# BBischof/ESRecsys

Measured on AMD Instinct MI355X. Metric: training pairs/sec, higher is better.
Workload: dtype f32; 1 GPU; inbatch: V=1000000 x D=128 fp32 tables, B=8192, sparse Adagrad; score_precision=auto -> f16x2, ids=uniform, parallelism=single

## Files before the change

esrecsys_amd/csrc/esr_inbatch2h.hip:

```cpp
#include "esr_inbatch_mfma.h"
#include <atomic>
#include <type_traits>
#include <time.h>

namespace esr {

typedef _Float16 f16x8 __attribute__((ext_vector_type(8)));
typedef _Float16 f16x2 __attribute__((ext_vector_type(2)));

constexpr int kHLseOff = 2 * kPlaneBytes;
constexpr int kHBufBytes = kHLseOff + 4 * 256;
constexpr float kHOptHead = 4.0f;
constexpr float kHOverflow = 60000.0f;
constexpr int kHBufs = 3;
constexpr float kHPexp = 14.0f;
constexpr float kHBoundSafe = 14.0f;
constexpr int kHScaleWords = 8;

#define H_MFMA(a, b, c) __builtin_amdgcn_mfma_f32_32x32x16_f16((a), (b), (c), 0, 0, 0)
#define H_SB() __builtin_amdgcn_sched_barrier(0)
#define H_DMA_BARRIER()                                 \
  {                                                     \
    asm volatile("s_waitcnt vmcnt(0)" ::: "memory");    \
    __syncthreads();                                    \
// ... 219 lines not shown
    const float4 f = rowsrc_load4(X, grow, d0 + 4 * q);
    v[4 * q] = f.x; v[4 * q + 1] = f.y; v[4 * q + 2] = f.z; v[4 * q + 3] = f.w;
  }
  {
    float ss = 0.f;
#pragma unroll
    for (int e = 0; e < 16; ++e) ss = fmaf(v[e], v[e], ss);
    ss += __shfl_xor(ss, 1, 64);
    ss += __shfl_xor(ss, 2, 64);
    ss += __shfl_xor(ss, 4, 64);
    ss = fmaxf(ss, __shfl_xor(ss, 8, 64));
    ss = fmaxf(ss, __shfl_xor(ss, 16, 64));
    ss = fmaxf(ss, __shfl_xor(ss, 32, 64));
    if ((t & 63) == 0) nrm[((int64_t)blockIdx.y * gridDim.x + chunk) * 4 + (t >> 6)] = ss;
  }
  f16x8 p[2][2];
#pragma unroll
  for (int e = 0; e < 16; ++e) {
    const float xs = v[e] * mul;
    const _Float16 a = (_Float16)xs;
    const _Float16 b = (_Float16)(xs - (float)a);
    p[0][e >> 3][e & 7] = a;
    p[1][e >> 3][e & 7] = b;
  }
#pragma unroll
  for (int pl = 0; pl < 2; ++pl) {
    f16x8* dst = reinterpret_cast<f16x8*>(R + ((int64_t)pl * B + grow) * k3D + d0);
    dst[0] = p[pl][0];
    dst[1] = p[pl][1];
  }
}

constexpr unsigned long long kPollTicks = 300000000ull;
__device__ __forceinline__ unsigned amax_code(float amax) {
  if (!(amax > 0.f)) return 0u;
  if (!(amax < INFINITY)) return 255u;
  int x;
  frexpf(amax, &x);
  return (unsigned)min(max(x + 127, 1), 254);
}
__device__ __forceinline__ int scale_exp_code(unsigned code) {
  if (code == 0u || code == 255u) return 0;
  const int e = 14 - ((int)code - 127);
  return e < -100 ? -100 : (e > 100 ? 100 : e);
}

__global__ __launch_bounds__(256) void prepsplit2h_kernel(RowSrc X0, RowSrc X1, int64_t B, _Float16* __restrict__ R0,
                                                         _Float16* __restrict__ R1,
                                                         unsigned long long* __restrict__ ent,
                                                         unsigned long long token, float* __restrict__ diag,
                                                         float* __restrict__ nrm, float* __restrict__ sc,
                                                         unsigned long long* __restrict__ loss_acc,
                                                         int* __restrict__ flags, int nflags,
                                                         float* __restrict__ copy0, float* __restrict__ copy1,
                                                         unsigned* __restrict__ czero, int two_level) {
  __shared__ float red[8];
  __shared__ unsigned cred[8];
  const int t = threadIdx.x, chunk = blockIdx.x, nchunks = gridDim.x;
  if (chunk == 0 && t <= kLossWords) {
    loss_acc[t * 16] = 0ull;
    if (t == 0) loss_acc[8] = 0ull;
  }
  if (chunk == 1 || nchunks == 1)
    for (int i = t; i < nflags; i += 256) flags[i] = 0;
  if (czero && chunk == 0 && t < 16) czero[t] = 0u;
  const int row = t >> 3, d0 = (t & 7) * 16;
  const int64_t grow = (int64_t)chunk * 32 + row;
  float vq[16], vc[16];
  {
    const int64_t rq = X0.idx ? (int64_t)X0.idx[grow] : grow;
    const int64_t rc = X1.idx ? (int64_t)X1.idx[grow] : grow;
    RowSrc Y0 = X0, Y1 = X1;
    Y0.idx = nullptr; Y1.idx = nullptr;
#pragma unroll
    for (int q = 0; q < 4; ++q) {
      const float4 f = rowsrc_load4(Y0, rq, d0 + 4 * q);
      const float4 g = rowsrc_load4(Y1, rc, d0 + 4 * q);
      vq[4 * q] = f.x; vq[4 * q + 1] = f.y; vq[4 * q + 2] = f.z; vq[4 * q + 3] = f.w;
      vc[4 * q] = g.x; vc[4 * q + 1] = g.y; vc[4 * q + 2] = g.z; vc[4 * q + 3] = g.w;
      if (copy0 && d0 + 4 * q < X0.ld) *reinterpret_cast<float4*>(copy0 + grow * X0.ld + d0 + 4 * q) = f;
      if (copy1 && d0 + 4 * q < X1.ld) *reinterpret_cast<float4*>(copy1 + grow * X1.ld + d0 + 4 * q) = g;
    }
  }
  float mq = 0.f, mc = 0.f, dot = 0.f, ssq = 0.f, ssc = 0.f;
#pragma unroll
  for (int e = 0; e < 16; ++e) {
    mq = fmaxf(mq, fabsf(vq[e]));
    mc = fmaxf(mc, fabsf(vc[e]));
    dot = fmaf(vq[e], vc[e], dot);
    ssq = fmaf(vq[e], vq[e], ssq);
    ssc = fmaf(vc[e], vc[e], ssc);
  }
  dot += __shfl_xor(dot, 1, 64); dot += __shfl_xor(dot, 2, 64); dot += __shfl_xor(dot, 4, 64);
  ssq += __shfl_xor(ssq, 1, 64); ssq += __shfl_xor(ssq, 2, 64); ssq += __shfl_xor(ssq, 4, 64);
  ssc += __shfl_xor(ssc, 1, 64); ssc += __shfl_xor(ssc, 2, 64); ssc += __shfl_xor(ssc, 4, 64);
  if ((t & 7) == 0) diag[grow] = dot;
#pragma unroll
  for (int o = 8; o < 64; o <<= 1) {
    ssq = fmaxf(ssq, __shfl_xor(ssq, o, 64));
    ssc = fmaxf(ssc, __shfl_xor(ssc, o, 64));
  }
  if ((t & 63) == 0) {
    nrm[((int64_t)0 * nchunks + chunk) * 4 + (t >> 6)] = ssq;
    nrm[((int64_t)1 * nchunks + chunk) * 4 + (t >> 6)] = ssc;
  }
#pragma unroll
  for (int o = 32; o > 0; o >>= 1) {
    mq = fmaxf(mq, __shfl_xor(mq, o, 64));
    mc = fmaxf(mc, __shfl_xor(mc, o, 64));
  }
  if ((t & 63) == 0) { red[t >> 6] = mq; red[4 + (t >> 6)] = mc; }
  __syncthreads();
  if (t == 0) {
    mq = fmaxf(fmaxf(red[0], red[1]), fmaxf(red[2], red[3]));
    mc = fmaxf(fmaxf(red[4], red[5]), fmaxf(red[6], red[7]));
    __hip_atomic_store(&ent[chunk], (token << 16) | (unsigned long long)(amax_code(mq) << 8 | amax_code(mc)),
                       __ATOMIC_RELAXED, __HIP_MEMORY_SCOPE_AGENT);
  }
  unsigned cq = 0u, cc = 0u;
  bool timed_out = false;
  const unsigned long long t_start = __builtin_amdgcn_s_memrealtime();
  const bool gatherer = chunk == 0 || !two_level;
  for (int i = gatherer ? t : (t == 0 ? nchunks : nchunks + 1); i < (gatherer ? nchunks : nchunks + 1); i += 256) {
    unsigned long long v;
    while (((v = __hip_atomic_load(&ent[i], __ATOMIC_RELAXED, __HIP_MEMORY_SCOPE_AGENT)) >> 16) != token) {
      if (__builtin_amdgcn_s_memrealtime() - t_start > kPollTicks) { timed_out = true; break; }
      __builtin_amdgcn_s_sleep(4);
    }
    cq = max(cq, (unsigned)(v >> 8) & 255u);
    cc = max(cc, (unsigned)v & 255u);
  }
  if (timed_out) atomicOr(reinterpret_cast<unsigned*>(loss_acc + 8), 1u);
#pragma unroll
  for (int o = 32; o > 0; o >>= 1) {
    cq = max(cq, (unsigned)__shfl_xor((int)cq, o, 64));
    cc = max(cc, (unsigned)__shfl_xor((int)cc, o, 64));
  }
  if ((t & 63) == 0) { cred[t >> 6] = cq; cred[4 + (t >> 6)] = cc; }
  __syncthreads();
  cq = max(max(cred[0], cred[1]), max(cred[2], cred[3]));
  cc = max(max(cred[4], cred[5]), max(cred[6], cred[7]));
  if (two_level && chunk == 0 && t == 0)
    __hip_atomic_store(&ent[nchunks], (token << 16) | (unsigned long long)(cq << 8 | cc), __ATOMIC_RELAXED,
                       __HIP_MEMORY_SCOPE_AGENT);
  const int eq = scale_exp_code(cq), ec = scale_exp_code(cc);
  if (chunk == 0 && t == 0) {
    sc[0] = ldexpf(1.f, -(eq + ec));
    sc[1] = ldexpf(1.f, -ec);
    sc[2] = ldexpf(1.f, -(eq + (int)kHPexp));
    sc[3] = ldexpf(1.f, eq);
// ... 228 lines not shown
    _Pragma("unroll") for (int g_ = 0; g_ < 2; ++g_) {                                                    \
      const u32x4 u_ = {pw[q_][4 * g_], pw[q_][4 * g_ + 1], pw[q_][4 * g_ + 2], pw[q_][4 * g_ + 3]};      \
      pb[q_][g_] = __builtin_bit_cast(f16x8, u_);                                                         \
    }
#define H_O_PHASE(DMA_ON, DBUF)                                                                           \
  {                                                                                                       \
    H_PB();                                                                                               \
    H_TR_WAIT();     \
    H_SB(); H_O_ROW(1, 0, 0); H_SB(); H_O_G1(0, 3); if (DMA_ON) { H_DP(0, g0, DBUF); }                    \
    H_SB(); H_O_ROW(0, 1, 0); H_SB(); H_O_G1(3, 6); if (DMA_ON) { H_DP(1, g1, DBUF); }                    \
    H_SB(); H_O_ROW(0, 0, 0); H_SB(); H_O_G1(6, 8); if (DMA_ON) { H_DP(2, g2, DBUF); }                    \
    H_TR_WAIT();                                                                                          \
    H_SB(); H_O_ROW(1, 0, 1); H_SB(); if (DMA_ON) { H_DP(3, g3, DBUF); }                                  \
    H_SB(); H_O_ROW(0, 1, 1); H_SB();                                                                     \
    H_SB(); H_O_ROW(0, 0, 1); H_SB();                                                                     \
    if (DMA_ON) H_DMA_ADVANCE();                                                                          \
  }
#define H_TR_BASES(BUF)                                                                                   \
  {                                                                                                       \
    const uint32_t slot_ = (uint32_t)((BUF) - lds);                                                       \
    _Pragma("unroll") for (int db_ = 0; db_ < 4; ++db_) { trc_[db_][0] = trb_[db_][0] + slot_; trc_[db_][1] = trb_[db_][1] + slot_; } \
  }
#define H_TR_SETUP()                                                                                      \
  const int tr_a = (lane & 15) >> 2;                                                                      \
  const int tr_e = (2 * ((lane >> 4) & 1)) + ((lane & 3) >> 1), tr_low = (lane & 1) * 8;                  \
  const int tr_row0 = (4 * h + tr_a) * 256, tr_row1 = (4 * h + 8 + tr_a) * 256;                           \
  const int tr_l0 = ((tr_e ^ (h & 3)) << 4) | tr_low, tr_l1 = ((tr_e ^ ((h + 2) & 3)) << 4) | tr_low;     \
  uint32_t trb_[4][2], trc_[4][2];                                                                        \
  _Pragma("unroll") for (int db = 0; db < 4; ++db) {                                                      \
    trb_[db][0] = (uint32_t)(uintptr_t)(__attribute__((address_space(3))) const char*)lds + tr_row0 + (((db ^ tr_a) << 6) | tr_l0); \
    trb_[db][1] = (uint32_t)(uintptr_t)(__attribute__((address_space(3))) const char*)lds + tr_row1 + (((db ^ tr_a) << 6) | tr_l1); \
  }

template <int KIND>
__global__ ESR_NO_PK __launch_bounds__(256) __attribute__((amdgpu_waves_per_eu(2, 2))) void inbatch2h_q_kernel(const _Float16* __restrict__ Xr, const _Float16* __restrict__ Yr,
                                                         int64_t B, int nsplit, float sl2_in,
                                                         const float* __restrict__ sc, const float* __restrict__ ref,
                                                         int nsplit_ref, const float* __restrict__ diag, int mode,
                                                         int* __restrict__ flags, float* __restrict__ part_m,
                                                         float* __restrict__ part_O, float* __restrict__ part_l,
                                                         float* __restrict__ Pmat) {
  __shared__ __attribute__((aligned(16))) char lds[kHBufs * kHBufBytes];
  if (KIND == 1 && flags[blockIdx.x] == 0) return;
  H_TIMING_DECL();
  int t = threadIdx.x, lane = t & 63;
  const int w = __builtin_amdgcn_readfirstlane(t >> 6);
  int j = lane & 31, h = lane >> 5;
  H_TR_SETUP();
  const uint32_t lds32 = (uint32_t)(uintptr_t)(__attribute__((address_space(3))) const char*)lds;
  (void)lds32;
  const int ob = blockIdx.x / nsplit, split = blockIdx.x % nsplit;
  const int64_t xrow = (int64_t)ob * k3Owned + w * 32 + j;
  const int nc = (int)(B / k3Chunk) / nsplit;
  const int64_t c0 = (int64_t)split * nc;
  const int64_t nch = B / 32;
  const float sl2 = sl2_in * sc[0];

  char* pst_u = nullptr;
  const uint32_t pst_v = (uint32_t)((((j >> 3) * 16) + ((2 * h + ((j >> 2) & 1)) * 4) + (j & 3)) * 16);
#if defined(H_PROBE_Q_NOSTORE)
#define H_P_ST(M, V0, V1, V2, V3)
#else
#define H_P_ST(M, V0, V1, V2, V3) \
  __builtin_nontemporal_store(u32x4{(V0), (V1), (V2), (V3)}, reinterpret_cast<u32x4*>(pst_u + (M) * 1024 + pst_v))
#endif

  f32x16 acc[4];
  f32x2 l2 = {0.f, 0.f};
  int dpos = 0;
  const char* const baseY = reinterpret_cast<const char*>(Yr);
  uint32_t g0 = 0, g1 = 0, g2 = 0, g3 = 0;
  f16x8 bx[2][8];
#pragma unroll
  for (int p = 0; p < 2; ++p)
// ... 123 lines not shown
      const f16x2 pq = pk_f16(resid_lo(e0, pa), resid_hi(e1, pa));
      pw[0][s] = __builtin_bit_cast(uint32_t, pa);
      pw[1][s] = __builtin_bit_cast(uint32_t, pq);
    }
#pragma unroll
    for (int m2 = 0; m2 < 2; ++m2)
#pragma unroll
      for (int pl = 0; pl < 2; ++pl) {
        H_P_ST(2 * m2 + pl, pw[pl][4 * m2], pw[pl][4 * m2 + 1], pw[pl][4 * m2 + 2], pw[pl][4 * m2 + 3]);
      }
    H_O_PHASE(false, lds);
  }
  };
  if (KIND == 1) {
    sweep(std::true_type{});
  } else {
    sweep(std::false_type{});
    if (KIND == 2 && mode != 0 && __syncthreads_or((mode == 2 || !(emax <= kHOverflow)) ? 1 : 0)) {
      asm volatile("" : "+v"(t), "+v"(lane), "+v"(j), "+v"(h));
      sweep(std::true_type{});
    }
  }
#undef H_P_ST
  H_TIMING_WRITE(H_TIMING_Q);
  float* orow = part_O + ((int64_t)split * B + xrow) * k3D;
#pragma unroll
  for (int db = 0; db < 4; ++db)
#pragma unroll
    for (int q = 0; q < 4; ++q)
      *reinterpret_cast<float4*>(orow + 32 * db + 8 * q + 4 * h) =
          make_float4(acc[db][4 * q], acc[db][4 * q + 1], acc[db][4 * q + 2], acc[db][4 * q + 3]);
  const float l = l2[0] + l2[1];
  const float ltot = l + __shfl_xor(l, 32, 64);
  if (h == 0) part_l[(int64_t)split * B + xrow] = ltot;
  if (KIND == 0 && (mode == 2 || !(emax <= kHOverflow))) flags[blockIdx.x] = 1;
}

template <int K>
__device__ __forceinline__ uint32_t dmah8_off0(int64_t B, int64_t chunk, int t) {
  const int row = t >> 4, seg = (t & 15) ^ swz16(row);
  return (uint32_t)((((int64_t)K * B + chunk * 32 + row) * k3D + seg * 8) * 2);
}
constexpr int kH1Waves = 8, kH1Owned = 32 * kH1Waves;
constexpr int kH1BufBytes = kPlaneBytes + kH1Waves * 256;
#define H1_DP(K, G, BUF) dmah_piece<K>(baseY, G, (BUF), w)
#define H1_DMA_REF(BUF)                                                                                   \
  __builtin_amdgcn_global_load_lds((gptr_t)(ref + (c0 + dpos) * 32 + (lane & 31)),                        \
                                   (lptr_t)((BUF) + kPlaneBytes + w * 256), 4, 0, 0)
#define H1_DMA_ADVANCE()                                                                   \
  {                                                                                        \
    const uint32_t step_ = (dpos + 1 == nc) ? (uint32_t)(8192 - nc * 8192) : 8192u;        \
    dpos = (dpos + 1 == nc) ? 0 : dpos + 1;                                                \
    g0 += step_;                                                                           \
  }
#define H1_DMA_CHUNK(BUF) { if (!QSIDE) { H1_DMA_REF(BUF); } H1_DP(0, g0, BUF); H1_DMA_ADVANCE(); }
#define H1_LOAD_REFS(BUF)                                                                                 \
  if (!QSIDE) {                                                                                           \
    f16x8 raw_[4];                                                                                        \
    _Pragma("unroll") for (int m_ = 0; m_ < 4; ++m_)                                                      \
      raw_[m_] = lds_b128<0>(lds32 + (uint32_t)((BUF) - lds) + (uint32_t)(kPlaneBytes + w * 256 + (8 * m_ + 4 * h) * 4)); \
    H_TR_WAIT();                                                                                          \
    _Pragma("unroll") for (int m_ = 0; m_ < 4; ++m_) {                                                    \
      const float4 lv_ = __builtin_bit_cast(float4, raw_[m_]);                                            \
      rf[4 * m_] = kHPexp - lv_.x; rf[4 * m_ + 1] = kHPexp - lv_.y;                                       \
      rf[4 * m_ + 2] = kHPexp - lv_.z; rf[4 * m_ + 3] = kHPexp - lv_.w;                                   \
    }                                                                                                     \
  }
// ... 641 lines not shown
                                                   float* __restrict__ lse_nat = nullptr) {
  const int64_t row = (int64_t)blockIdx.x * 256 + threadIdx.x;
  if (row >= B) return;
  float pm[8], pl[8];
#pragma unroll
  for (int s = 0; s < 8; ++s) {
    pm[s] = -INFINITY; pl[s] = 0.f;
    if (s < nsplit) {
      pm[s] = part_m[(int64_t)s * B + row];
      pl[s] = part_l[(int64_t)s * B + row];
    }
  }
  float M = pm[0], L = 0.f;
  float wt[8];
#pragma unroll
  for (int s = 1; s < 8; ++s) M = fmaxf(M, pm[s]);
#pragma unroll
  for (int s = 0; s < 8; ++s) {
    wt[s] = pm[s] == M ? 1.f : __builtin_amdgcn_exp2f(pm[s] - M);
    L = __fmaf_rn(pl[s], wt[s], L);
  }
  const float invL1 = __fdiv_rn(1.0f, L);
#pragma unroll
  for (int s = 0; s < 8; ++s)
    if (s < nsplit) fac[(int64_t)s * B + row] = __fmul_rn(__fmul_rn(invL1, invl_scale), wt[s]);
  if (lse2) {
    const float l2v = __fadd_rn(M, __builtin_amdgcn_logf(L));
    lse2[row] = l2v;
    if (lse_nat) lse_nat[row] = l2v * k3Ln2;
  }
}

constexpr int kCtExpShift = 11;
__global__ __launch_bounds__(256) void facscale2h_kernel(RowSrc X, int64_t B, int nsplit,
                                                        const float* __restrict__ part_m,
                                                        const float* __restrict__ part_l, float invl_scale,
                                                        const float* __restrict__ sc, float* __restrict__ fac,
                                                        float* __restrict__ lse2, float* __restrict__ lse_nat,
                                                        _Float16* __restrict__ Yt, int* __restrict__ cflags) {
  const int t = threadIdx.x, chunk = blockIdx.x;
  const int row = t >> 3, sl = t & 7, d0 = sl * 16;
  const int64_t grow = (int64_t)chunk * 32 + row;
  float v[16];
  {
    const int64_t r = X.idx ? (int64_t)X.idx[grow] : grow;
    RowSrc Y0 = X;
    Y0.idx = nullptr;
#pragma unroll
    for (int q = 0; q < 4; ++q) {
      const float4 f = rowsrc_load4(Y0, r, d0 + 4 * q);
      v[4 * q] = f.x; v[4 * q + 1] = f.y; v[4 * q + 2] = f.z; v[4 * q + 3] = f.w;
    }
  }
  const float pm_l = sl < nsplit ? part_m[(int64_t)sl * B + grow] : -INFINITY;
  const float pl_l = sl < nsplit ? part_l[(int64_t)sl * B + grow] : 0.f;
  float pm[8], pl[8];
  const int lane0 = (t & 63) & ~7;
#pragma unroll
  for (int s = 0; s < 8; ++s) {
    pm[s] = __shfl(pm_l, lane0 + s, 64);
    pl[s] = __shfl(pl_l, lane0 + s, 64);
  }
  float M = pm[0], L = 0.f;
  float wt[8];
#pragma unroll
  for (int s = 1; s < 8; ++s) M = fmaxf(M, pm[s]);
#pragma unroll
  for (int s = 0; s < 8; ++s) {
    wt[s] = pm[s] == M ? 1.f : __builtin_amdgcn_exp2f(pm[s] - M);
    L = __fmaf_rn(pl[s], wt[s], L);
  }
  const float invL1 = __fdiv_rn(1.0f, L);
  const float f1 = __fmul_rn(invL1, invl_scale);
  float wmine = 1.f;
#pragma unroll
  for (int s = 0; s < 8; ++s) wmine = s == sl ? wt[s] : wmine;
  const float fs = __fmul_rn(f1, wmine);
  if (sl < nsplit) {
    fac[(int64_t)sl * B + grow] = fs;
    if (fs != f1) cflags[sl] = 1;
  }
  if (sl == 0 && lse2) {
    const float l2v = __fadd_rn(M, __builtin_amdgcn_logf(L));
    lse2[grow] = l2v;
    if (lse_nat) lse_nat[grow] = l2v * k3Ln2;
  }
  const float mul = sc[3] * ldexpf(1.f, -kCtExpShift);
  float m = 0.f;
  f16x8 p[2][2];
#pragma unroll
  for (int e = 0; e < 16; ++e) {
    const float xs = __fmul_rn(v[e], f1) * mul;
    m = fmaxf(m, fabsf(xs));
    const _Float16 a = (_Float16)xs;
    const _Float16 b = (_Float16)(xs - (float)a);
    p[0][e >> 3][e & 7] = a;
    p[1][e >> 3][e & 7] = b;
  }
  m = fmaxf(m, __shfl_xor(m, 1, 64));
  m = fmaxf(m, __shfl_xor(m, 2, 64));
  m = fmaxf(m, __shfl_xor(m, 4, 64));
  if (sl < nsplit && (!(m < 60000.f) || (f1 != 0.f && m < kCtLive))) cflags[sl] = 1;
#pragma unroll
  for (int pl2 = 0; pl2 < 2; ++pl2) {
    f16x8* dst = reinterpret_cast<f16x8*>(Yt + ((int64_t)pl2 * B + grow) * k3D + d0);
    dst[0] = p[pl2][0];
    dst[1] = p[pl2][1];
  }
}

struct InbatchHWs {
  _Float16 *Qh, *Ch;
  float *part_O, *part_O2, *fac_side, *Qcopy, *Ccopy, *part_m, *part_mr, *part_l, *lse2, *fac, *Pmat, *nrm, *amax, *sc, *diag;
  int* flags;
  unsigned long long* loss_acc;
  unsigned long long* ent;
  _Float16* Qt;
  unsigned* czero;
  int* cflags;
};
constexpr int64_t kHMaxB = 16384;

static size_t inbatch2h_ws_layout(int64_t B, char* base, InbatchHWs* ws) {
  size_t off = 0;
  auto take = [&](size_t bytes) {
    char* p = base ? base + off : nullptr;
    off += align_up(bytes, 256);
    return p;
  };
  const size_t planes = (size_t)2 * B * k3D * 2;
  InbatchHWs w;
  w.Qh = (_Float16*)take(planes);
  w.Ch = (_Float16*)take(planes);
  w.part_O = (float*)take((size_t)8 * B * k3D * 4);
  w.part_O2 = (float*)take((size_t)8 * B * k3D * 4);
  w.fac_side = (float*)take((size_t)8 * B * 4);
  w.Qcopy = (float*)take((size_t)B * k3D * 4);
  w.Ccopy = (float*)take((size_t)B * k3D * 4);
  w.part_m = (float*)take((size_t)8 * B * 4);
  w.part_mr = (float*)take((size_t)8 * B * 4);
  w.part_l = (float*)take((size_t)8 * B * 4);
  w.lse2 = (float*)take((size_t)B * 4);
  w.fac = (float*)take((size_t)8 * B * 4);
  w.diag = (float*)take((size_t)B * 4);
  w.flags = (int*)take((size_t)8 * (B / k3Owned) * sizeof(int));
  w.Pmat = (float*)take((size_t)B * B * 4);
  w.loss_acc = (unsigned long long*)take(sizeof(unsigned long long) * 16 * (1 + kLossWords));
  w.nrm = (float*)take((size_t)2 * (B / k3Chunk) * 4 * sizeof(float));
  w.amax = (float*)take((size_t)2 * (B / k3Chunk) * sizeof(float));
  w.sc = (float*)take(kHScaleWords * sizeof(float));
  w.ent = (unsigned long long*)take((size_t)(B / k3Chunk + 1) * sizeof(unsigned long long));
  w.Qt = (_Float16*)take(planes);
  w.czero = (unsigned*)take(16 * sizeof(unsigned));
  w.cflags = reinterpret_cast<int*>(w.czero ? w.czero + 8 : nullptr);
  if (ws) *ws = w;
  return off;
}

static int inbatch2h_nsplit(int64_t B, int per_cu) {
  const int64_t owned_blocks = B / k3Owned, nchunks = B / k3Chunk;
  int best = 1;
  for (int s = 1; s <= 8; ++s)
    if (nchunks % s == 0 && owned_blocks * s <= 320 * per_cu) best = s;
  return best;
}

struct InbatchUpdate {
  void* tables[2];
  float* accums[2];
  int64_t row_offsets[3];
  int dtype;
  const int32_t* sorted_vids;
  const int32_t* perm;
  float* grad_rows;
  float lr, eps;
  bool skip_long;
};

int inbatch_merge_update(void* const* tables, float* const* accums, const int64_t* row_offsets, int dtype,
                         const int32_t* sorted_vids, const int32_t* perm, const InbatchMergeArgs& a, float lr, float eps,
                         hipStream_t st);
int sparse_adagrad_range(void* const* tables, float* const* accums, const int64_t* row_offsets, int ntables, int dtype,
                         int D, const int32_t* sorted_vids, const int32_t* perm, int64_t n, float* grad_rows, float lr,
                         float eps, bool skip_long, hipStream_t st);

static bool inbatch_events(hipEvent_t* fork, hipEvent_t* join) {
  constexpr int kMaxDev = 16;
// ... 65 lines not shown
  const int pc_blocks = (int)cdiv(B, kCtOwned);
  int nsplit_c = 1;
  for (int sp = 1; sp <= 8; ++sp)
    if (nchunks % sp == 0 && pc_blocks * sp <= 320) nsplit_c = sp;
  const int grid_c = pc_blocks * nsplit_c;
  const int grid_q = (int)(B / k3Owned) * nsplit_q;
  const int mgrid = (int)std::min<int64_t>(k3MergeBlocks, cdiv(B, kBlock / 32));
  const char* refe = getenv("ESR_IB2H_REF");
  const int mode = (refe && refe[0] == 'r' && refe[1] == 'o') ? 0 : ((refe && refe[0] == 'r' && refe[1] == 'e') ? 2 : 1);
  const char* fe = getenv("ESR_IB2H_FUSED");
  const bool fused = !(fe && fe[0] == '0') && mode != 0;
  int nsplit_r = 1;
  hipEvent_t ev_fork = nullptr, ev_join = nullptr;
  const char* b16e = getenv("ESR_IB2H_BF16");
  const bool one_plane = fused && ((Qs.bf16 && Cs.bf16 && !(b16e && b16e[0] == 't')) || (b16e && b16e[0] == 'f'));
  const bool overlapped = fused && !one_plane && side != nullptr && side != st && inbatch_events(&ev_fork, &ev_join);
  const char* mue = getenv("ESR_IB2H_MERGE_UPDATE");
  const bool merge_upd = fused && !overlapped && upd != nullptr && upd->skip_long && D == k3D && Qs.ld == k3D &&
                         Cs.ld == k3D && !(mue && mue[0] == '0');
  auto merging_update = [&](int nsplit_of_c, const float* part_O_of_c) -> int {
    InbatchMergeArgs a;
    a.part_O[0] = ws.part_O; a.part_O[1] = part_O_of_c;
    a.nsplit[0] = nsplit_q; a.nsplit[1] = nsplit_of_c;
    a.oscale[0] = ws.sc + 1; a.oscale[1] = ws.sc + 2;
    a.partner[0] = ws.Ccopy; a.partner[1] = ws.Qcopy;
    a.part_m = ws.part_m; a.part_l = ws.part_l;
    a.B = B;
    a.scale = scale; a.lam = regularization; a.inv_bs = inv_bs;
    a.loss_acc = ws.loss_acc; a.loss_scale = 1.0 / (double)batch_size; a.loss_out = loss;
    a.zero_words = ws.ent; a.nzero = nchunks + 1;
    return inbatch_merge_update(upd->tables, upd->accums, upd->row_offsets, upd->dtype, upd->sorted_vids, upd->perm, a,
                                upd->lr, upd->eps, st);
  };
  if (fused) {
    static std::atomic<unsigned long long> call_seq{0};
    static const unsigned long long seed =
        (unsigned long long)(uintptr_t)&call_seq ^ (unsigned long long)time(nullptr) * 0x9E3779B97F4A7C15ull;
    unsigned long long z = seed + 0x9E3779B97F4A7C15ull * (call_seq.fetch_add(1) + 1);
    z = (z ^ (z >> 30)) * 0xBF58476D1CE4E5B9ull;
    z = (z ^ (z >> 27)) * 0x94D049BB133111EBull;
    const unsigned long long token = ((z ^ (z >> 31)) >> 16) | 1ull;
    const char* tle = getenv("ESR_IB2H_POLL");
    const int two_level = (tle && tle[0] == 'f') ? 0 : 1;
    ESR_KT("prepsplit2h_kernel", st,
           hipLaunchKernelGGL(prepsplit2h_kernel, dim3(nchunks), dim3(256), 0, st, Qs, Cs, B, ws.Qh, ws.Ch, ws.ent, token,
                              ws.diag, ws.nrm, ws.sc, ws.loss_acc, ws.flags, grid_q, (overlapped || merge_upd) ? ws.Qcopy : (float*)nullptr,
                              (overlapped || merge_upd) ? ws.Ccopy : (float*)nullptr, ws.czero, two_level));
    if (one_plane) {
      const int blocks1 = (int)cdiv(B, kH1Owned);
      int nsplit_1 = 1;
      for (int sp = 1; sp <= 8; ++sp)
        if (nchunks % sp == 0 && blocks1 * sp <= 320) nsplit_1 = sp;
      const int nsplit_q = nsplit_1, grid_q = blocks1 * nsplit_1;
      const char* dbg1h = getenv("ESR_IB1H_DBG");
      if (dbg1h && dbg1h[0] == '1') {
        hipLaunchKernelGGL((inbatch1h_kernel<true, 1>), dim3(grid_q), dim3(512), 0, st, (const _Float16*)ws.Qh,
                           (const _Float16*)ws.Ch, B, nsplit_q, sl2, (const float*)ws.sc, (const float*)ws.diag,
                           (const float*)nullptr, mode, ws.part_m, ws.part_O, ws.part_l);
      } else
      ESR_KT("inbatch1h_kernel_q", st,
             hipLaunchKernelGGL((inbatch1h_kernel<true>), dim3(grid_q), dim3(512), 0, st, (const _Float16*)ws.Qh,
                                (const _Float16*)ws.Ch, B, nsplit_q, sl2, (const float*)ws.sc, (const float*)ws.diag,
                                (const float*)nullptr, mode, ws.part_m, ws.part_O, ws.part_l));
      if (merge_upd) {
        ESR_KT("fac2h_kernel", st,
               hipLaunchKernelGGL(fac2h_kernel, dim3((unsigned)cdiv(B, 256)), dim3(256), 0, st, B, nsplit_q,
                                  (const float*)ws.part_m, (const float*)ws.part_l, ldexpf(1.f, (int)kHPexp), ws.fac,
                                  ws.lse2, lse));
      } else
      ESR_KT("inbatch3_merge_kernel_q", st,
             hipLaunchKernelGGL((inbatch3_merge_kernel<true>), dim3(mgrid), dim3(kBlock), 0, st, Qs, Cs, gq_rows, B,
                                nsplit_q, (const float*)ws.part_O, (const float*)ws.part_m, (const float*)ws.part_l, scale,
                                regularization, inv_bs, ws.lse2, lse, gQ, ws.loss_acc, 1.0 / (double)batch_size, loss,
                                (float*)nullptr, (const float*)(ws.sc + 1), ldexpf(1.f, (int)kHPexp), ws.fac));
      float* const part_O_1c = merge_upd ? ws.part_O2 : ws.part_O;
      if (dbg1h && (dbg1h[0] == '1' || dbg1h[0] == '2')) {
        hipLaunchKernelGGL((inbatch1h_kernel<false, 1>), dim3(grid_q), dim3(512), 0, st, (const _Float16*)ws.Ch,
                           (const _Float16*)ws.Qh, B, nsplit_q, sl2, (const float*)ws.sc, (const float*)nullptr,
                           (const float*)ws.lse2, mode, (float*)nullptr, part_O_1c, (float*)nullptr);
      } else
      ESR_KT("inbatch1h_kernel_c", st,
             hipLaunchKernelGGL((inbatch1h_kernel<false>), dim3(grid_q), dim3(512), 0, st, (const _Float16*)ws.Ch,
                                (const _Float16*)ws.Qh, B, nsplit_q, sl2, (const float*)ws.sc, (const float*)nullptr,
                                (const float*)ws.lse2, mode, (float*)nullptr, part_O_1c, (float*)nullptr));
      if (merge_upd) return merging_update(nsplit_q, part_O_1c);
      ESR_KT("inbatch3_merge_kernel_c", st,
             hipLaunchKernelGGL((inbatch3_merge_kernel<false>), dim3(mgrid), dim3(kBlock), 0, st, Cs, Qs, gc_rows, B,
                                nsplit_q, (const float*)ws.part_O, (const float*)ws.part_m, (const float*)ws.part_l, scale,
                                regularization, inv_bs, ws.lse2, (float*)nullptr, gC, ws.loss_acc,
                                1.0 / (double)batch_size, loss, (float*)nullptr, (const float*)(ws.sc + 2), 1.0f,
                                (float*)nullptr, ws.ent, nchunks + 1));
      if (upd) {
        const int rc = sparse_adagrad_range(upd->tables, upd->accums, upd->row_offsets, 2, upd->dtype, D, upd->sorted_vids,
                                            upd->perm, 2 * B, upd->grad_rows, upd->lr, upd->eps, upd->skip_long, st);
        if (rc != ESR_OK) return rc;
      }
      return check_launch(who);
    }
    ESR_KT("inbatch2h_q_kernel", st,
           hipLaunchKernelGGL((inbatch2h_q_kernel<2>), dim3(grid_q), dim3(256), 0, st, (const _Float16*)ws.Qh,
                              (const _Float16*)ws.Ch, B, nsplit_q, sl2, (const float*)ws.sc, (const float*)ws.part_mr, 1,
                              (const float*)ws.diag, mode, ws.flags, ws.part_m, ws.part_O, ws.part_l, ws.Pmat));
  } else {
  ESR_KT("prep2h_kernel", st, hipLaunchKernelGGL(prep2h_kernel, dim3(nchunks), dim3(256), 0, st, Qs, Cs, ws.amax, ws.diag));
  ESR_KT("split2h_kernel", st,
         hipLaunchKernelGGL(split2h_kernel, dim3(nchunks, 2), dim3(256), 0, st, Qs, Cs, B, ws.Qh, ws.Ch,
                            (const float*)ws.amax, ws.nrm, ws.sc, ws.loss_acc, ws.flags, grid_q));
  if (mode == 0) {
    const int rm_blocks = (int)cdiv(B, kHRmOwned);
    for (int sp = 1; sp <= 8; ++sp)
      if (nchunks % sp == 0 && rm_blocks * sp <= 320) nsplit_r = sp;
    ESR_KT("rowmax2h_kernel", st,
           hipLaunchKernelGGL(rowmax2h_kernel, dim3(rm_blocks * nsplit_r), dim3(256), 0, st, (const _Float16*)ws.Qh,
                              (const _Float16*)ws.Ch, B, nsplit_r, sl2, (const float*)ws.nrm, (const float*)ws.sc,
                              ws.part_mr));
  }
  {
    ESR_KT("inbatch2h_q_kernel", st,
           hipLaunchKernelGGL((inbatch2h_q_kernel<0>), dim3(grid_q), dim3(256), 0, st, (const _Float16*)ws.Qh,
                              (const _Float16*)ws.Ch, B, nsplit_q, sl2, (const float*)ws.sc, (const float*)ws.part_mr,
                              nsplit_r, (const float*)ws.diag, mode, ws.flags, ws.part_m, ws.part_O, ws.part_l, ws.Pmat));
    if (mode != 0)
      ESR_KT("inbatch2h_q_kernel_redo", st,
             hipLaunchKernelGGL((inbatch2h_q_kernel<1>), dim3(grid_q), dim3(256), 0, st, (const _Float16*)ws.Qh,
                                (const _Float16*)ws.Ch, B, nsplit_q, sl2, (const float*)ws.sc, (const float*)ws.part_mr,
                                nsplit_r, (const float*)ws.diag, mode, ws.flags, ws.part_m, ws.part_O, ws.part_l, ws.Pmat));
  }
  }
  hipStream_t st_q = overlapped ? side : st;
  float* const part_O_c = (overlapped || merge_upd) ? ws.part_O2 : ws.part_O;
  const RowSrc Qm = overlapped ? RowSrc{ws.Qcopy, nullptr, 0, Qs.ld} : Qs;
  const RowSrc Cm = overlapped ? RowSrc{ws.Ccopy, nullptr, 0, Cs.ld} : Cs;
  const int nc_q = nchunks / nsplit_q;
  const char* pcm = getenv("ESR_IB2H_PC");
  const int force_general = (!fused || (pcm && pcm[0] == 'g')) ? 1 : 0;
  if (overlapped) {
    if (hipEventRecord(ev_fork, st) != hipSuccess || hipStreamWaitEvent(side, ev_fork, 0) != hipSuccess) {
      set_error("%s: could not fork the side stream", who);
      return ESR_ELAUNCH;
    }
  }
  if (!force_general)
    ESR_KT("facscale2h_kernel", st,
           hipLaunchKernelGGL(facscale2h_kernel, dim3(nchunks), dim3(256), 0, st,
                              (overlapped || merge_upd) ? RowSrc{ws.Qcopy, nullptr, 0, Qs.ld} : Qs, B, nsplit_q,
                              (const float*)ws.part_m, (const float*)ws.part_l, ldexpf(1.f, (int)kHPexp),
                              (const float*)ws.sc, ws.fac, merge_upd ? ws.lse2 : (float*)nullptr,
                              merge_upd ? lse : (float*)nullptr, ws.Qt, ws.cflags));
  else if (overlapped || merge_upd)
    ESR_KT("fac2h_kernel", st,
           hipLaunchKernelGGL(fac2h_kernel, dim3((unsigned)cdiv(B, 256)), dim3(256), 0, st, B, nsplit_q,
                              (const float*)ws.part_m, (const float*)ws.part_l, ldexpf(1.f, (int)kHPexp), ws.fac,
                              merge_upd ? ws.lse2 : (float*)nullptr, merge_upd ? lse : (float*)nullptr));
  if (!merge_upd)
  ESR_KT("inbatch3_merge_kernel_q", st_q,
         hipLaunchKernelGGL((inbatch3_merge_kernel<true>), dim3(mgrid), dim3(kBlock), 0, st_q, Qm, Cm, gq_rows, B, nsplit_q,
                            (const float*)ws.part_O, (const float*)ws.part_m, (const float*)ws.part_l, scale,
                            regularization, inv_bs, ws.lse2, lse, gQ, ws.loss_acc, 1.0 / (double)batch_size, loss,
                            (float*)nullptr, (const float*)(ws.sc + 1), ldexpf(1.f, (int)kHPexp),
                            overlapped ? ws.fac_side : ws.fac));
  if (overlapped) {
    if (upd) {
      const int rc = sparse_adagrad_range(upd->tables, upd->accums, upd->row_offsets, 2, upd->dtype, D, upd->sorted_vids,
                                          upd->perm, B, upd->grad_rows, upd->lr, upd->eps, upd->skip_long, side);
      if (rc != ESR_OK) return rc;
    }
    if (hipEventRecord(ev_join, side) != hipSuccess) {
      set_error("%s: could not record the join event", who);
      return ESR_ELAUNCH;
    }
  }
  ESR_KT("inbatch2h_pct_kernel", st,
         hipLaunchKernelGGL(inbatch2h_pct_kernel, dim3(grid_c), dim3(512), 0, st, (const _Float16*)ws.Qt,
                            (const _Float16*)ws.Qh, B, nsplit_c, (const float*)ws.fac, nc_q, (const char*)ws.Pmat,
                            ldexpf(1.f, kCtExpShift), (const int*)ws.cflags, force_general, part_O_c));
// ... 138 lines not shown
```

Baseline: 38.60 million pairs/s.

## Fuse facscale into q-kernel epilogue via arrival counter; defer prep copies

Adds an optional epilogue to the in-batch q kernel. Each split block publishes its partial max and sum, then bumps a per-row-group arrival counter, and the last block to arrive computes the softmax factors and the scaled f16 Q planes itself. This removes the separate facscale kernel launch. Independently, the prep kernel now writes its fp32 row copies after publishing the amax entry instead of during the loads, which shortens the path to the cross-block poll but keeps the values live in registers longer. The fused epilogue is opt-in through an environment variable and adds zeroed counter words to the workspace.

Result: no change. 38.63 million pairs/s, median of 2 (+0.1%).

```diff
diff --git a/esrecsys_amd/csrc/esr_inbatch2h.hip b/esrecsys_amd/csrc/esr_inbatch2h.hip
--- a/esrecsys_amd/csrc/esr_inbatch2h.hip
+++ b/esrecsys_amd/csrc/esr_inbatch2h.hip
@@ -275,6 +275,9 @@
 }
 
 constexpr unsigned long long kPollTicks = 300000000ull;
+constexpr int64_t kHMaxB = 16384;
+constexpr int kHZeroWords = 16 + (int)(kHMaxB / k3Owned);
+static_assert(kHZeroWords <= 256, "one thread per zeroed word");
 __device__ __forceinline__ unsigned amax_code(float amax) {
   if (!(amax > 0.f)) return 0u;
   if (!(amax < INFINITY)) return 255u;
@@ -296,7 +299,7 @@
                                                          unsigned long long* __restrict__ loss_acc,
                                                          int* __restrict__ flags, int nflags,
                                                          float* __restrict__ copy0, float* __restrict__ copy1,
-                                                         unsigned* __restrict__ czero, int two_level) {
+                                                         unsigned* __restrict__ czero, int two_level, int copy_late) {
   __shared__ float red[8];
   __shared__ unsigned cred[8];
   const int t = threadIdx.x, chunk = blockIdx.x, nchunks = gridDim.x;
@@ -306,7 +309,7 @@
   }
   if (chunk == 1 || nchunks == 1)
     for (int i = t; i < nflags; i += 256) flags[i] = 0;
-  if (czero && chunk == 0 && t < 16) czero[t] = 0u;
+  if (czero && chunk == 0 && t < kHZeroWords) czero[t] = 0u;
   const int row = t >> 3, d0 = (t & 7) * 16;
   const int64_t grow = (int64_t)chunk * 32 + row;
   float vq[16], vc[16];
@@ -321,8 +324,10 @@
       const float4 g = rowsrc_load4(Y1, rc, d0 + 4 * q);
       vq[4 * q] = f.x; vq[4 * q + 1] = f.y; vq[4 * q + 2] = f.z; vq[4 * q + 3] = f.w;
       vc[4 * q] = g.x; vc[4 * q + 1] = g.y; vc[4 * q + 2] = g.z; vc[4 * q + 3] = g.w;
-      if (copy0 && d0 + 4 * q < X0.ld) *reinterpret_cast<float4*>(copy0 + grow * X0.ld + d0 + 4 * q) = f;
-      if (copy1 && d0 + 4 * q < X1.ld) *reinterpret_cast<float4*>(copy1 + grow * X1.ld + d0 + 4 * q) = g;
+      if (!copy_late) {
+        if (copy0 && d0 + 4 * q < X0.ld) *reinterpret_cast<float4*>(copy0 + grow * X0.ld + d0 + 4 * q) = f;
+        if (copy1 && d0 + 4 * q < X1.ld) *reinterpret_cast<float4*>(copy1 + grow * X1.ld + d0 + 4 * q) = g;
+      }
     }
   }
   float mq = 0.f, mc = 0.f, dot = 0.f, ssq = 0.f, ssc = 0.f;
@@ -359,6 +364,17 @@
     mc = fmaxf(fmaxf(red[4], red[5]), fmaxf(red[6], red[7]));
     __hip_atomic_store(&ent[chunk], (token << 16) | (unsigned long long)(amax_code(mq) << 8 | amax_code(mc)),
                        __ATOMIC_RELAXED, __HIP_MEMORY_SCOPE_AGENT);
+  }
+  if (copy_late) {
+#pragma unroll
+    for (int q = 0; q < 4; ++q) {
+      if (copy0 && d0 + 4 * q < X0.ld)
+        *reinterpret_cast<float4*>(copy0 + grow * X0.ld + d0 + 4 * q) =
+            make_float4(vq[4 * q], vq[4 * q + 1], vq[4 * q + 2], vq[4 * q + 3]);
+      if (copy1 && d0 + 4 * q < X1.ld)
+        *reinterpret_cast<float4*>(copy1 + grow * X1.ld + d0 + 4 * q) =
+            make_float4(vc[4 * q], vc[4 * q + 1], vc[4 * q + 2], vc[4 * q + 3]);
+    }
   }
   unsigned cq = 0u, cc = 0u;
   bool timed_out = false;
@@ -653,14 +669,24 @@
     trb_[db][1] = (uint32_t)(uintptr_t)(__attribute__((address_space(3))) const char*)lds + tr_row1 + (((db ^ tr_a) << 6) | tr_l1); \
   }
 
-template <int KIND>
+struct FacEpi {
+  unsigned* arrive;
+  const float* X;
+  float invl_scale;
+  float *fac, *lse2, *lse_nat;
+  _Float16* Yt;
+  int* cflags;
+};
+static __device__ void facscale2h_block(FacEpi e, int t, int ob, int64_t B, int nsplit, const float* part_m,
+                                        const float* part_l, const float* __restrict__ sc);
+template <int KIND, bool EPI = false>
 __global__ ESR_NO_PK __launch_bounds__(256) __attribute__((amdgpu_waves_per_eu(2, 2))) void inbatch2h_q_kernel(const _Float16* __restrict__ Xr, const _Float16* __restrict__ Yr,
                                                          int64_t B, int nsplit, float sl2_in,
                                                          const float* __restrict__ sc, const float* __restrict__ ref,
                                                          int nsplit_ref, const float* __restrict__ diag, int mode,
                                                          int* __restrict__ flags, float* __restrict__ part_m,
                                                          float* __restrict__ part_O, float* __restrict__ part_l,
-                                                         float* __restrict__ Pmat) {
+                                                         float* __restrict__ Pmat, FacEpi epi) {
   __shared__ __attribute__((aligned(16))) char lds[kHBufs * kHBufBytes];
   if (KIND == 1 && flags[blockIdx.x] == 0) return;
   H_TIMING_DECL();
@@ -850,7 +876,22 @@
           make_float4(acc[db][4 * q], acc[db][4 * q + 1], acc[db][4 * q + 2], acc[db][4 * q + 3]);
   const float l = l2[0] + l2[1];
   const float ltot = l + __shfl_xor(l, 32, 64);
-  if (h == 0) part_l[(int64_t)split * B + xrow] = ltot;
+  const bool arrive = KIND == 2 && EPI;
+  const int te = w * 64 + h * 32 + j;
+  unsigned arrived = 0u;
+  if (arrive) {
+    if (h == 0) {
+      __hip_atomic_store(&part_m[(int64_t)split * B + xrow], -nrefv[0], __ATOMIC_RELAXED, __HIP_MEMORY_SCOPE_AGENT);
+      __hip_atomic_store(&part_l[(int64_t)split * B + xrow], ltot, __ATOMIC_RELAXED, __HIP_MEMORY_SCOPE_AGENT);
+    }
+    asm volatile("s_waitcnt vmcnt(0)" ::: "memory");
+    __syncthreads();
+    if (te == 0) arrived = __hip_atomic_fetch_add(&epi.arrive[ob], 1u, __ATOMIC_RELAXED, __HIP_MEMORY_SCOPE_AGENT) + 1u;
+  } else if (h == 0) {
+    part_l[(int64_t)split * B + xrow] = ltot;
+  }
+  if (arrive && __syncthreads_or(arrived == (unsigned)nsplit ? 1 : 0))
+    facscale2h_block(epi, te, ob, B, nsplit, part_m, part_l, sc);
   if (KIND == 0 && (mode == 2 || !(emax <= kHOverflow))) flags[blockIdx.x] = 1;
 }
 
@@ -1558,6 +1599,67 @@
 }
 
 constexpr int kCtExpShift = 11;
+__device__ __forceinline__ void facscale2h_row(const float (&v)[16], float pm_l, float pl_l, int t, int sl, int64_t grow,
+                                               int64_t B, int nsplit, float invl_scale, const float* __restrict__ sc,
+                                               float* __restrict__ fac, float* __restrict__ lse2,
+                                               float* __restrict__ lse_nat, _Float16* __restrict__ Yt,
+                                               int* __restrict__ cflags) {
+  const int d0 = sl * 16;
+  float pm[8], pl[8];
+  const int lane0 = (t & 63) & ~7;
+#pragma unroll
+  for (int s = 0; s < 8; ++s) {
+    pm[s] = __shfl(pm_l, lane0 + s, 64);
+    pl[s] = __shfl(pl_l, lane0 + s, 64);
+  }
+  float M = pm[0], L = 0.f;
+  float wt[8];
+#pragma unroll
+  for (int s = 1; s < 8; ++s) M = fmaxf(M, pm[s]);
+#pragma unroll
+  for (int s = 0; s < 8; ++s) {
+    wt[s] = pm[s] == M ? 1.f : __builtin_amdgcn_exp2f(pm[s] - M);
+    L = __fmaf_rn(pl[s], wt[s], L);
+  }
+  const float invL1 = __fdiv_rn(1.0f, L);
+  const float f1 = __fmul_rn(invL1, invl_scale);
+  float wmine = 1.f;
+#pragma unroll
+  for (int s = 0; s < 8; ++s) wmine = s == sl ? wt[s] : wmine;
+  const float fs = __fmul_rn(f1, wmine);
+  if (sl < nsplit) {
+    fac[(int64_t)sl * B + grow] = fs;
+    if (fs != f1) cflags[sl] = 1;
+  }
+  if (sl == 0 && lse2) {
+    const float l2v = __fadd_rn(M, __builtin_amdgcn_logf(L));
+    lse2[grow] = l2v;
+    if (lse_nat) lse_nat[grow] = l2v * k3Ln2;
+  }
+  const float mul = sc[3] * ldexpf(1.f, -kCtExpShift);
+  float m = 0.f;
+  f16x8 p[2][2];
+#pragma unroll
+  for (int e = 0; e < 16; ++e) {
+    const float xs = __fmul_rn(v[e], f1) * mul;
+    m = fmaxf(m, fabsf(xs));
+    const _Float16 a = (_Float16)xs;
+    const _Float16 b = (_Float16)(xs - (float)a);
+    p[0][e >> 3][e & 7] = a;
+    p[1][e >> 3][e & 7] = b;
+  }
+  m = fmaxf(m, __shfl_xor(m, 1, 64));
+  m = fmaxf(m, __shfl_xor(m, 2, 64));
+  m = fmaxf(m, __shfl_xor(m, 4, 64));
+  if (sl < nsplit && (!(m < 60000.f) || (f1 != 0.f && m < kCtLive))) cflags[sl] = 1;
+#pragma unroll
+  for (int pl2 = 0; pl2 < 2; ++pl2) {
+    f16x8* dst = reinterpret_cast<f16x8*>(Yt + ((int64_t)pl2 * B + grow) * k3D + d0);
+    dst[0] = p[pl2][0];
+    dst[1] = p[pl2][1];
+  }
+}
+
 __global__ __launch_bounds__(256) void facscale2h_kernel(RowSrc X, int64_t B, int nsplit,
                                                         const float* __restrict__ part_m,
                                                         const float* __restrict__ part_l, float invl_scale,
@@ -1580,59 +1682,31 @@
   }
   const float pm_l = sl < nsplit ? part_m[(int64_t)sl * B + grow] : -INFINITY;
   const float pl_l = sl < nsplit ? part_l[(int64_t)sl * B + grow] : 0.f;
-  float pm[8], pl[8];
-  const int lane0 = (t & 63) & ~7;
-#pragma unroll
-  for (int s = 0; s < 8; ++s) {
-    pm[s] = __shfl(pm_l, lane0 + s, 64);
-    pl[s] = __shfl(pl_l, lane0 + s, 64);
-  }
-  float M = pm[0], L = 0.f;
-  float wt[8];
-#pragma unroll
-  for (int s = 1; s < 8; ++s) M = fmaxf(M, pm[s]);
-#pragma unroll
-  for (int s = 0; s < 8; ++s) {
-    wt[s] = pm[s] == M ? 1.f : __builtin_amdgcn_exp2f(pm[s] - M);
-    L = __fmaf_rn(pl[s], wt[s], L);
-  }
-  const float invL1 = __fdiv_rn(1.0f, L);
-  const float f1 = __fmul_rn(invL1, invl_scale);
-  float wmine = 1.f;
-#pragma unroll
-  for (int s = 0; s < 8; ++s) wmine = s == sl ? wt[s] : wmine;
-  const float fs = __fmul_rn(f1, wmine);
-  if (sl < nsplit) {
-    fac[(int64_t)sl * B + grow] = fs;
-    if (fs != f1) cflags[sl] = 1;
-  }
-  if (sl == 0 && lse2) {
-    const float l2v = __fadd_rn(M, __builtin_amdgcn_logf(L));
-    lse2[grow] = l2v;
-    if (lse_nat) lse_nat[grow] = l2v * k3Ln2;
-  }
-  const float mul = sc[3] * ldexpf(1.f, -kCtExpShift);
-  float m = 0.f;
-  f16x8 p[2][2];
-#pragma unroll
-  for (int e = 0; e < 16; ++e) {
-    const float xs = __fmul_rn(v[e], f1) * mul;
-    m = fmaxf(m, fabsf(xs));
-    const _Float16 a = (_Float16)xs;
-    const _Float16 b = (_Float16)(xs - (float)a);
-    p[0][e >> 3][e & 7] = a;
-    p[1][e >> 3][e & 7] = b;
-  }
-  m = fmaxf(m, __shfl_xor(m, 1, 64));
-  m = fmaxf(m, __shfl_xor(m, 2, 64));
-  m = fmaxf(m, __shfl_xor(m, 4, 64));
-  if (sl < nsplit && (!(m < 60000.f) || (f1 != 0.f && m < kCtLive))) cflags[sl] = 1;
-#pragma unroll
-  for (int pl2 = 0; pl2 < 2; ++pl2) {
-    f16x8* dst = reinterpret_cast<f16x8*>(Yt + ((int64_t)pl2 * B + grow) * k3D + d0);
-    dst[0] = p[pl2][0];
-    dst[1] = p[pl2][1];
-  }
+  facscale2h_row(v, pm_l, pl_l, t, sl, grow, B, nsplit, invl_scale, sc, fac, lse2, lse_nat, Yt, cflags);
+}
+
+static __device__ void facscale2h_block(FacEpi e, int t, int ob, int64_t B, int nsplit, const float* part_m,
+                                        const float* part_l, const float* __restrict__ sc) {
+  const int sl = t & 7;
+  float v[4][16], pm_l[4], pl_l[4];
+#pragma unroll
+  for (int r = 0; r < 4; ++r) {
+    const int64_t grow = (int64_t)ob * k3Owned + r * 32 + (t >> 3);
+#pragma unroll
+    for (int q = 0; q < 4; ++q) {
+      const float4 f = *reinterpret_cast<const float4*>(e.X + grow * k3D + sl * 16 + 4 * q);
+      v[r][4 * q] = f.x; v[r][4 * q + 1] = f.y; v[r][4 * q + 2] = f.z; v[r][4 * q + 3] = f.w;
+    }
+    pm_l[r] = -INFINITY; pl_l[r] = 0.f;
+    if (sl < nsplit) {
+      pm_l[r] = __hip_atomic_load(&part_m[(int64_t)sl * B + grow], __ATOMIC_RELAXED, __HIP_MEMORY_SCOPE_AGENT);
+      pl_l[r] = __hip_atomic_load(&part_l[(int64_t)sl * B + grow], __ATOMIC_RELAXED, __HIP_MEMORY_SCOPE_AGENT);
+    }
+  }
+#pragma unroll
+  for (int r = 0; r < 4; ++r)
+    facscale2h_row(v[r], pm_l[r], pl_l[r], t, sl, (int64_t)ob * k3Owned + r * 32 + (t >> 3), B, nsplit, e.invl_scale, sc,
+                   e.fac, e.lse2, e.lse_nat, e.Yt, e.cflags);
 }
 
 struct InbatchHWs {
@@ -1644,8 +1718,8 @@
   _Float16* Qt;
   unsigned* czero;
   int* cflags;
+  unsigned* arrive;
 };
-constexpr int64_t kHMaxB = 16384;
 
 static size_t inbatch2h_ws_layout(int64_t B, char* base, InbatchHWs* ws) {
   size_t off = 0;
@@ -1677,8 +1751,9 @@
   w.sc = (float*)take(kHScaleWords * sizeof(float));
   w.ent = (unsigned long long*)take((size_t)(B / k3Chunk + 1) * sizeof(unsigned long long));
   w.Qt = (_Float16*)take(planes);
-  w.czero = (unsigned*)take(16 * sizeof(unsigned));
+  w.czero = (unsigned*)take(kHZeroWords * sizeof(unsigned));
   w.cflags = reinterpret_cast<int*>(w.czero ? w.czero + 8 : nullptr);
+  w.arrive = w.czero ? w.czero + 16 : nullptr;
   if (ws) *ws = w;
   return off;
 }
@@ -1810,6 +1885,15 @@
     return inbatch_merge_update(upd->tables, upd->accums, upd->row_offsets, upd->dtype, upd->sorted_vids, upd->perm, a,
                                 upd->lr, upd->eps, st);
   };
+  const char* pcm = getenv("ESR_IB2H_PC");
+  const int force_general = (!fused || (pcm && pcm[0] == 'g')) ? 1 : 0;
+  const char* fse = getenv("ESR_IB2H_FACSCALE");
+  const bool fac_epilogue = merge_upd && !one_plane && !force_general && fse && fse[0] == 'e';
+  FacEpi epi{};
+  if (fac_epilogue) {
+    epi.arrive = ws.arrive; epi.X = ws.Qcopy; epi.invl_scale = ldexpf(1.f, (int)kHPexp);
+    epi.fac = ws.fac; epi.lse2 = ws.lse2; epi.lse_nat = lse; epi.Yt = ws.Qt; epi.cflags = ws.cflags;
+  }
   if (fused) {
     static std::atomic<unsigned long long> call_seq{0};
     static const unsigned long long seed =
@@ -1820,10 +1904,12 @@
     const unsigned long long token = ((z ^ (z >> 31)) >> 16) | 1ull;
     const char* tle = getenv("ESR_IB2H_POLL");
     const int two_level = (tle && tle[0] == 'f') ? 0 : 1;
+    const char* cpe = getenv("ESR_IB2H_COPY");
+    const int copy_late = (cpe && cpe[0] == 'e') ? 0 : 1;
     ESR_KT("prepsplit2h_kernel", st,
            hipLaunchKernelGGL(prepsplit2h_kernel, dim3(nchunks), dim3(256), 0, st, Qs, Cs, B, ws.Qh, ws.Ch, ws.ent, token,
                               ws.diag, ws.nrm, ws.sc, ws.loss_acc, ws.flags, grid_q, (overlapped || merge_upd) ? ws.Qcopy : (float*)nullptr,
-                              (overlapped || merge_upd) ? ws.Ccopy : (float*)nullptr, ws.czero, two_level));
+                              (overlapped || merge_upd) ? ws.Ccopy : (float*)nullptr, ws.czero, two_level, copy_late));
     if (one_plane) {
       const int blocks1 = (int)cdiv(B, kH1Owned);
       int nsplit_1 = 1;
@@ -1875,10 +1961,16 @@
       }
       return check_launch(who);
     }
+    if (fac_epilogue)
+      ESR_KT("inbatch2h_q_kernel", st,
+             hipLaunchKernelGGL((inbatch2h_q_kernel<2, true>), dim3(grid_q), dim3(256), 0, st, (const _Float16*)ws.Qh,
+                                (const _Float16*)ws.Ch, B, nsplit_q, sl2, (const float*)ws.sc, (const float*)ws.part_mr, 1,
+                                (const float*)ws.diag, mode, ws.flags, ws.part_m, ws.part_O, ws.part_l, ws.Pmat, epi));
+    else
     ESR_KT("inbatch2h_q_kernel", st,
            hipLaunchKernelGGL((inbatch2h_q_kernel<2>), dim3(grid_q), dim3(256), 0, st, (const _Float16*)ws.Qh,
                               (const _Float16*)ws.Ch, B, nsplit_q, sl2, (const float*)ws.sc, (const float*)ws.part_mr, 1,
-                              (const float*)ws.diag, mode, ws.flags, ws.part_m, ws.part_O, ws.part_l, ws.Pmat));
+                              (const float*)ws.diag, mode, ws.flags, ws.part_m, ws.part_O, ws.part_l, ws.Pmat, epi));
   } else {
   ESR_KT("prep2h_kernel", st, hipLaunchKernelGGL(prep2h_kernel, dim3(nchunks), dim3(256), 0, st, Qs, Cs, ws.amax, ws.diag));
   ESR_KT("split2h_kernel", st,
@@ -1897,12 +1989,12 @@
     ESR_KT("inbatch2h_q_kernel", st,
            hipLaunchKernelGGL((inbatch2h_q_kernel<0>), dim3(grid_q), dim3(256), 0, st, (const _Float16*)ws.Qh,
                               (const _Float16*)ws.Ch, B, nsplit_q, sl2, (const float*)ws.sc, (const float*)ws.part_mr,
-                              nsplit_r, (const float*)ws.diag, mode, ws.flags, ws.part_m, ws.part_O, ws.part_l, ws.Pmat));
+                              nsplit_r, (const float*)ws.diag, mode, ws.flags, ws.part_m, ws.part_O, ws.part_l, ws.Pmat, FacEpi{}));
     if (mode != 0)
       ESR_KT("inbatch2h_q_kernel_redo", st,
              hipLaunchKernelGGL((inbatch2h_q_kernel<1>), dim3(grid_q), dim3(256), 0, st, (const _Float16*)ws.Qh,
                                 (const _Float16*)ws.Ch, B, nsplit_q, sl2, (const float*)ws.sc, (const float*)ws.part_mr,
-                                nsplit_r, (const float*)ws.diag, mode, ws.flags, ws.part_m, ws.part_O, ws.part_l, ws.Pmat));
+                                nsplit_r, (const float*)ws.diag, mode, ws.flags, ws.part_m, ws.part_O, ws.part_l, ws.Pmat, FacEpi{}));
   }
   }
   hipStream_t st_q = overlapped ? side : st;
@@ -1910,15 +2002,14 @@
   const RowSrc Qm = overlapped ? RowSrc{ws.Qcopy, nullptr, 0, Qs.ld} : Qs;
   const RowSrc Cm = overlapped ? RowSrc{ws.Ccopy, nullptr, 0, Cs.ld} : Cs;
   const int nc_q = nchunks / nsplit_q;
-  const char* pcm = getenv("ESR_IB2H_PC");
-  const int force_general = (!fused || (pcm && pcm[0] == 'g')) ? 1 : 0;
   if (overlapped) {
     if (hipEventRecord(ev_fork, st) != hipSuccess || hipStreamWaitEvent(side, ev_fork, 0) != hipSuccess) {
       set_error("%s: could not fork the side stream", who);
       return ESR_ELAUNCH;
     }
   }
-  if (!force_general)
+  if (fac_epilogue) {
+  } else if (!force_general)
     ESR_KT("facscale2h_kernel", st,
            hipLaunchKernelGGL(facscale2h_kernel, dim3(nchunks), dim3(256), 0, st,
                               (overlapped || merge_upd) ? RowSrc{ws.Qcopy, nullptr, 0, Qs.ld} : Qs, B, nsplit_q,
```
